# uio-bmi/compairr

Hardware: AMD Instinct MI355X
Metric: query sequences/sec for --matrix d=1, 10M-vs-10M CDR3aa (higher is better)
Workload: dtype u64; 1 GPU; synthetic 10M-vs-10M CDR3aa, d=1 substitutions only, V/J matched; queries_total=10000000, queries_this_gpu=10000000, reference_sequences=10000000, matrix_checksum=fc9769626ca2bcf2c84e8473864b8853

## Files before the change

compairr_amd/csrc/compairr_hip.hip:

```cpp
#include "context.h"
#include "kernels_sliced.h"
#include "kernels_rows.h"
#include "kernels_pairs2.h"
#include "select.h"

#include <algorithm>
#include <cmath>
#include <cstdio>
#include <cstdlib>
#include <cstring>
#include <new>
#include <mutex>
#include <string>
#include <thread>
#include <vector>

using namespace cmpr;

std::string &cmpr_create_error()
{
  static thread_local std::string e;
  return e;
}

// ... 226 lines not shown
    if (c->ring_k0[i]) (void)hipEventDestroy(c->ring_k0[i]);
    if (c->ring_km[i]) (void)hipEventDestroy(c->ring_km[i]);
    if (c->ring_k1[i]) (void)hipEventDestroy(c->ring_k1[i]);
  }
  if (c->ev_stop) (void)hipEventDestroy(c->ev_stop);
  if (c->ev_usage) (void)hipEventDestroy(c->ev_usage);
  if (c->d_usage) (void)hipFree(c->d_usage);
  if (c->h_usage) (void)hipHostFree(c->h_usage);
  c->arena_a.release();
  c->arena_b.release();
  if (c->stage_host) (void)hipHostFree(c->stage_host);
  if (c->h_sizes) (void)hipHostFree(c->h_sizes);
  for (uint32_t i = 0; i < cmpr_context::NCOPY_EV; i++)
    if (c->ev_copy[i]) (void)hipEventDestroy(c->ev_copy[i]);
  for (hipEvent_t e : c->ev_layout)
    if (e) (void)hipEventDestroy(e);
  if (c->copy_stream) (void)hipStreamDestroy(c->copy_stream);
  if (c->stream) (void)hipStreamDestroy(c->stream);
  delete c;
}

extern "C" const char *cmpr_last_error(const cmpr_context *c)
{
  return c ? c->err.c_str() : cmpr_create_error().c_str();
}

extern "C" uint32_t cmpr_rows(const cmpr_context *c) { return c ? c->R1 : 0; }
extern "C" uint32_t cmpr_cols(const cmpr_context *c) { return c ? c->R2 : 0; }

namespace {
enum TunLock { LOCK_NEVER, LOCK_REF, LOCK_QUERIES };
enum : unsigned { T_NO_PLAN = 1, T_WRITE_ONLY = 2 };

struct Tunable {
  const char *name;
  int64_t cmpr_context::*field;
  int64_t lo, hi;
  TunLock lock;
  unsigned flags;
  const char *range_msg;
  bool (*also)(const cmpr_context *, int64_t);
  void (*after)(cmpr_context *, int64_t);
  const char *lock_msg;
};

bool power_of_two(const cmpr_context *, int64_t v) { return (v & (v - 1)) == 0; }
bool not_zero(const cmpr_context *, int64_t v) { return v != 0; }
bool class_res_fits(const cmpr_context *c, int64_t v) { return v <= (int64_t)max_class_res((uint32_t)c->opt.alphabet_size); }
void force_waves(cmpr_context *c, int64_t) { c->waves_per_block_forced = true; }
void pretend_never_overflows(cmpr_context *c, int64_t v)
{
  c->force_no_redo = v != 0;
  c->usage_pending = false;
}
const char SHARD_RANGE[] = "work_shard_count must be 1..65535, work_shard_index 0..count-1",
           SHARD_LOCK[] = "set the work shard before cmpr_set_queries";
const char BOOL_RANGE[] = " must be 0 or 1", AUTO_RANGE[] = " must be -1 (auto), 0 or 1";

#define F(field) &cmpr_context::field
const Tunable TUNABLES[] = {
  {"blocks_per_cu", F(blocks_per_cu), 1, 16, LOCK_NEVER, 0, " must be 1..16"},
  {"variant", F(variant), -1, 2, LOCK_REF, 0, " must be -1 (default), 0, 1 or 2"},
  {"class_residues", F(class_residues), -1, 8, LOCK_REF, 0,
   " must be -1..4 (amino acids; four: variant 2, d = 1, else three) / -1..8 (nucleotides)", class_res_fits},
  {"class_anchor", F(class_anchor), -1, 65535, LOCK_REF, 0, " must be -1..65535"},
  {"heavy_threshold", F(heavy_threshold), -1, INT64_MAX, LOCK_REF, 0, " must be >= -1"},
  {"slice_words_log2", F(slice_words_log2), -1, 13, LOCK_REF, 0, " must be -1 (default) or 1..13", not_zero},
  {"chunk_tiles", F(chunk_tiles), 0, 512, LOCK_QUERIES, 0, " must be 0..512"},
#ifdef CMPR_ABLATION
  {"debug", F(debug), INT64_MIN, INT64_MAX, LOCK_NEVER, 0, ""},
#else
  {"debug", F(debug), 1, 0, LOCK_NEVER, 0, "the debug switches exist only in a -DCMPR_ABLATION build"},
#endif
  {"host_threads", F(host_threads), 1, 256, LOCK_NEVER, T_NO_PLAN, " must be 1..256"},
  {"table_log2_delta", F(table_log2_delta), 0, 3, LOCK_REF, 0, " must be 0..3"},
  {"part_buckets_log2", F(part_buckets_log2), 2, 30, LOCK_REF, 0, " must be 2..30"},
  {"deferred_resolve", F(deferred_resolve), 0, 1, LOCK_NEVER, 0, BOOL_RANGE},
  {"d2_pairs", F(d2_pairs), -1, 1, LOCK_REF, 0, AUTO_RANGE},
  {"d2_buffers", F(d2_buffers), 1, 2, LOCK_REF, 0, " must be 1 or 2"},
  {"chunk_deal", F(chunk_deal), 0, 1, LOCK_NEVER, 0, " must be 0 (static) or 1 (by a counter)"},
  {"narrow_upload", F(narrow_upload), -1, 1, LOCK_NEVER, T_NO_PLAN, AUTO_RANGE},
  {"item_wg", F(item_wg), 0, 1, LOCK_NEVER, T_NO_PLAN, BOOL_RANGE},
  {"layout_recompute", F(layout_recompute), 0, 1, LOCK_NEVER, T_NO_PLAN, BOOL_RANGE},
  {"layout_timing", F(layout_timing), 0, 1, LOCK_NEVER, T_NO_PLAN, BOOL_RANGE},
  {"layout_zob_lds", F(layout_zob_lds), 0, 1, LOCK_NEVER, T_NO_PLAN | T_WRITE_ONLY, BOOL_RANGE},
  {"record_tiles", F(record_tiles), 0, 2, LOCK_QUERIES, T_NO_PLAN, " must be 0, 1 or 2"},
  {"assume_never_overflows", nullptr, INT64_MIN, INT64_MAX, LOCK_NEVER, T_NO_PLAN | T_WRITE_ONLY, "", nullptr, pretend_never_overflows},
  {"dedup_tag_bits", F(dedup_tag_bits), 0, 32, LOCK_NEVER, T_NO_PLAN, " must be 0..32"},
  {"resolve_blocks_per_cu", F(resolve_blocks_per_cu), 1, 8, LOCK_NEVER, 0, " must be 1..8"},
  {"pos_segments", F(pos_segments), 1, 256, LOCK_QUERIES, 0, " must be a power of two, 1..256", power_of_two},
  {"pos_grow", F(pos_grow), -1, 1, LOCK_NEVER, 0, AUTO_RANGE},
  {"pos_capacity", F(pos_capacity), 0, INT64_MAX, LOCK_QUERIES, 0, " must be >= 0"},
  {"work_shard_count", F(work_shard_count), 1, 65535, LOCK_QUERIES, 0, SHARD_RANGE, nullptr, nullptr, SHARD_LOCK},
  {"work_shard_index", F(work_shard_index), 0, 65535, LOCK_QUERIES, 0, SHARD_RANGE, nullptr, nullptr, SHARD_LOCK},
  {"small_slice_tiles", F(small_slice_tiles), 0, 64, LOCK_QUERIES, 0, " must be 0..64"},
  {"sub2_items", F(sub2_items), -1, 1, LOCK_QUERIES, 0, " must be -1 (default), 0 or 1"},
  {"class_rows_unstaged", F(class_rows_unstaged), 0, 1, LOCK_QUERIES, 0, BOOL_RANGE},
  {"waves_per_block", F(waves_per_block), 4, 16, LOCK_QUERIES, 0, " must be 4, 8 or 16", power_of_two, force_waves},
  {"bloom_bits_log2_delta", F(bloom_log2_delta), -4, 4, LOCK_REF, 0, " must be -4..4"},
  {"slice_pages", F(slice_pages), -1, (int64_t)PAGE_E_MAX, LOCK_REF, 0, " must be -1..3"},
  {"page_budget", F(page_budget), 0, 1 << 24, LOCK_REF, 0, " must be 0..2^24"},
  {"bucket_bitmap", F(bucket_bitmap), -1, 1, LOCK_NEVER, 0, AUTO_RANGE},
  {"fill_slices", F(fill_slices), 0, 1, LOCK_REF, 0, BOOL_RANGE},
  {"direct_slices_log2", F(direct_slices_log2), -1, 12, LOCK_NEVER, 0, " must be -1 (auto) or 0..12"},
  {"row_filter_x16", F(row_filter_x16), 8, 128, LOCK_REF, 0, " must be 8..128 (sixteenths of a byte per entry)"},
};
#undef F

const Tunable *find_tunable(const char *name)
{
  for (const Tunable &t : TUNABLES)
    if (!strcmp(t.name, name))
      return &t;
  return nullptr;
}

bool in_range(const cmpr_context *c, const Tunable &t, int64_t value)
{
  return value >= t.lo && value <= t.hi && (!t.also || t.also(c, value));
}

void store_tunable(cmpr_context *c, const Tunable &t, int64_t value)
{
  if (t.field)
    c->*t.field = value;
  if (t.after)
    t.after(c, value);
}

void tunable_from_environment(cmpr_context *c, const char *variable, const char *name)
{
  const char *e = getenv(variable);
  const Tunable *t = find_tunable(name);
  if (e && t && in_range(c, *t, atoi(e)))
    store_tunable(c, *t, atoi(e));
}

}

extern "C" int cmpr_set_tunable(cmpr_context *c, const char *name, int64_t value)
{
  if (!c || !name)
    return CMPR_EINVAL;
  const Tunable *t = find_tunable(name);
  if (!t)
    return fail(c, CMPR_EINVAL, std::string("unknown tunable: ") + name);
  if (!in_range(c, *t, value))
    return fail(c, CMPR_EINVAL, t->range_msg[0] == ' ' ? t->name + std::string(t->range_msg) : t->range_msg);
  if (t->lock == LOCK_REF ? c->have_ref : t->lock == LOCK_QUERIES && c->have_q)
    return fail(c, CMPR_ESTATE, t->lock_msg ? t->lock_msg : std::string("set ") + t->name + " before " +
                                (t->lock == LOCK_REF ? "cmpr_set_reference" : "cmpr_set_queries"));
  store_tunable(c, *t, value);
  if (!(t->flags & T_NO_PLAN)) {
    invalidate_plan(c);
    c->usage_pending = c->never_overflows = false;
  }
  return CMPR_OK;
}

extern "C" int cmpr_get_tunable(cmpr_context *c, const char *name, int64_t *value)
{
  if (!c || !name || !value)
    return CMPR_EINVAL;
  std::string n(name);
  if (n == "variant") *value = c->have_ref ? (c->rows ? 2 : c->sliced ? 1 : 0) : c->variant;
  else if (n == "bloom_bits_log2_delta") {
// ... 1028 lines not shown
```

compairr_amd/csrc/context.h:

```cpp
#ifndef COMPAIRR_AMD_CONTEXT_H
#define COMPAIRR_AMD_CONTEXT_H

#include "../../include/compairr_hip.h"
#include "kernels.h"

#include "select.h"

#include <functional>
#include <map>
#include <set>
#include <string>
#include <vector>

struct SplitMix64 {
  uint64_t s;
  explicit SplitMix64(uint64_t seed) : s(seed) {}
  uint64_t next()
  {
    uint64_t z = (s += 0x9e3779b97f4a7c15ull);
    z = (z ^ (z >> 30)) * 0xbf58476d1ce4e5b9ull;
    z = (z ^ (z >> 27)) * 0x94d049bb133111ebull;
    return z ^ (z >> 31);
  }
};
// ... 54 lines not shown
  std::function<int()> finish;
};

struct RouteState {
  bool     valid = false;
  uint64_t n = 0, first_index = 0, total_records = 0;
  uint32_t n_dest = 0, record_bytes = 0;
  unsigned long long counts[64] = {};
  std::vector<double> rep_totals;
  const uint8_t  *res = nullptr;
  const uint64_t *off = nullptr, *cnt = nullptr;
  const uint32_t *v = nullptr, *j = nullptr, *rep = nullptr;
  const uint32_t *mask_lo = nullptr, *mask_hi = nullptr;
  unsigned long long *dest = nullptr;
};

struct RefPart {
  uint64_t              first = 0, n = 0;
  uint64_t              slots = 0;
  DevBuf<uint64_t>      bloom;
  DevBuf<unsigned char> rec;
  DevBuf<uint32_t>      bmap;
  void release()
  {
    bloom.release();
    rec.release();
    bmap.release();
  }
};

struct cmpr_context {
  cmpr_options opt{};
  int          device = 0;
  int          cus = 256;
  hipStream_t  stream = nullptr;
  hipEvent_t   ev_stop = nullptr;
  static const uint32_t TIME_RING = 64;
  hipEvent_t   ring_k0[TIME_RING] = {}, ring_km[TIME_RING] = {}, ring_k1[TIME_RING] = {};
  hipEvent_t   ring_start[TIME_RING] = {};
  hipEvent_t   ring_mid[TIME_RING] = {};
  uint64_t     calls = 0;
  hipEvent_t   ev_k0 = nullptr, ev_km = nullptr, ev_k1 = nullptr;
  bool         events_valid = false;
  bool         stop_is_k1 = false;
  hipEvent_t   pending_launch = nullptr;
  std::string  err;

  int64_t blocks_per_cu = 8;
  int64_t variant = -1;
  int64_t bloom_log2_delta = -100;
  int64_t row_filter_x16 = 32;
  int64_t slice_pages = -1;
  int64_t page_budget = 0;
  int64_t bucket_bitmap = -1;
  int64_t direct_slices_log2 = -1;
  int64_t fill_slices = 1;
  int64_t class_residues = -1;
  int64_t class_anchor = -1;
  int64_t heavy_threshold = -1;
  int64_t chunk_tiles = 0;
  int64_t waves_per_block = 8;
  bool    sub2_active = false;
  int64_t sub2_items = -1;
  int64_t work_shard_index = 0;
  int64_t work_shard_count = 1;
  int64_t small_slice_tiles = 0;
  int64_t class_rows_unstaged = 0;
  int64_t host_threads = 0;
  int64_t table_log2_delta = 1;
  int64_t deferred_resolve = 1;
  int64_t chunk_deal = 1;
  int64_t pos_capacity = 0;
  int64_t pos_grow = -1;
  int64_t resolve_blocks_per_cu = 5;
  int64_t pos_segments = 64;
  bool    waves_per_block_forced = false;
  int64_t debug = 0;
  int64_t slice_words_log2 = -1;
  int64_t part_buckets_log2 = 30;
  int64_t d2_pairs = -1;
  int64_t d2_buffers = 1;
  int64_t narrow_upload = -1;
  int64_t item_wg = 1, layout_recompute = 1, layout_timing = 0;
  int64_t layout_zob_lds = 1;
  int64_t record_tiles = 1;
  int64_t dedup_tag_bits = 32;
  uint32_t chunk_cap = 0;

  bool                  sliced = false;
  bool                  rows = false;
  uint32_t              npasses = 1;
  SliceGeom             geom{};
  std::vector<uint32_t> ctab;
  DevBuf<uint32_t>      d_ctab;
  DevBuf<uint32_t>      page_tab;
  uint64_t              page_slices = 0;
  DevBuf<Chunk>         chunks;
  DevBuf<cmpr::TileRef> tile_refs;
  DevBuf<uint32_t>      small_tiles;
  uint32_t              nsmall = 0;
  uint32_t              nchunks = 0;

  uint32_t          zpos = 0;
  DevBuf<uint64_t>  zob;

  bool              have_ref = false;
  uint64_t          n2 = 0;
  uint32_t          R2 = 0, longest2 = 0;
  DevBuf<uint8_t>   res2;
  DevBuf<uint64_t>  off2, cnt2, bloom;
  DevBuf<uint32_t>  v2, j2, rep2;
  DevBuf<uint32_t>  bmap2;
  DevBuf<unsigned char> rec2;
  DevBuf<uint32_t>  voff2;
  uint64_t          slots = 0, bloom_words = 0;
  uint32_t          nparts = 1;
  uint64_t          part0_n = 0;
  std::vector<RefPart> xparts;
  DevBuf<unsigned long long> stats_acc;

  bool              have_q = false;
  bool              routed = false;
  RouteState        route;
  uint64_t          n1 = 0;
  uint32_t          R1 = 0, ntiles = 0;
  DevBuf<TileDesc>  tiles;
  uint32_t          nmain_tiles = 0;
  DevBuf<uint32_t>  qres, qv, qj;
  DevBuf<uint64_t>  qgh;
  DevBuf<uint64_t>  qhins, qhdel;
  DevBuf<uint16_t>  qlen;
  DevBuf<uint32_t>  qck;
  DevBuf<cmpr::QueryRec> qrec;
  DevBuf<cmpr::ItemRec> items;
  DevBuf<uint32_t>  slice_items;
  DevBuf<cmpr::ResPack> cpk;
  DevBuf<cmpr::ResPack> qpk;
  bool              d2pairs = false;
  uint64_t          algorithmic_bytes = 0;
  double            max_cell_bound = 0;
  std::vector<double> tot1, tot2;

  DevBuf<unsigned long long> matrix;
  DevBuf<double>             matrix_f64;
  DevBuf<PosEntry>           pos_buf;
  DevBuf<unsigned long long> pos_ctr;
  unsigned long long        *ctr_cur = nullptr, *ctr_other = nullptr;
  bool                       ctr_clean = false;
  unsigned long long        *d_usage = nullptr;
  unsigned long long        *h_usage = nullptr;
  hipEvent_t                 ev_usage = nullptr;
  bool                       usage_pending = false, never_overflows = false;
  uint32_t                   usage_grid = 0, usage_nw = 0, safe_grid = 0, safe_nw = 0;
  bool                       last_without_redo = false;
  bool                       force_no_redo = false;
  bool                       async_unchecked = false, async_overflowed = false;
  hipStream_t                last_stream = nullptr;
  bool                       have_last_stream = false;
  DevArena                   arena_a, arena_b;
  void                      *stage_host = nullptr;
  size_t                     stage_host_bytes = 0;
  hipStream_t                copy_stream = nullptr;
  static const uint32_t      NCOPY_EV = 4;
  hipEvent_t                 ev_copy[NCOPY_EV] = {};
  double                     layout_upload_ms = 0, layout_tail_ms = 0, layout_total_ms = 0;
  bool                       rec_tiles = false;
// ... 159 lines not shown
```

compairr_amd/csrc/query_layout.hip:

```cpp
#include "context.h"
#include "kernels_sliced.h"

#include <hipcub/hipcub.hpp>

#include <algorithm>
#include <atomic>
#include <chrono>
#include <cstdio>
#include <cstdlib>
#include <cstring>
#include <thread>

using namespace cmpr;

namespace {

constexpr uint32_t MAXP = 1 + MAX_CLASS_RES;
constexpr uint32_t FOREIGN_SLICES_LOG2 = 12;

enum : uint32_t { VERR_OFFSETS = 1, VERR_LONG = 2, VERR_REP = 3, VERR_GENE = 4, VERR_COUNT = 5,
                  VERR_RESIDUE = 6, VERR_TOO_LONG = 7, VERR_OFFSETS0 = 8 };

struct SliceTot {
  uint32_t tiles, chunks, small, list;
// ... 804 lines not shown
    }
    for (uint32_t gl = gl_end; gl < Q.per_slice; gl++) {
      const uint32_t L = Q.longest - gl;
      const uint32_t n = c[gl];
      const uint32_t nt = (n + WAVE - 1) / WAVE;
      if (WRITE) {
        const uint64_t g = bucket * Q.per_slice + gl;
        Q.base_g[pi][g] = (tile_base + ntiles) * WAVE;
        if (pi == 0)
          Q.tfirst_g[g] = tile_base + ntiles;
      }
      for (uint32_t k = 0; k < nt; k++) {
        const uint32_t nv = min((uint32_t)WAVE, n - k * WAVE);
        if (WRITE) {
          TileDesc td;
          td.len = L;
          td.nvalid = nv;
          td.res_base = (uint32_t)(Q.res0[pi] + at.res + res);
          td.pass = pass;
          td.slice = (uint32_t)sl;
          td.k = tile_k;
          Q.tiles[tile_base + ntiles + k] = td;
        }
        res += pi == 0 ? (unsigned long long)((L + 3) / 4) * WAVE : (unsigned long long)WAVE;
        work_lens += (uint64_t)(L + 1) * nv;
      }
      ntiles += nt;
    }
  }
  uint32_t nchunks = 0, nsmall = 0, nlist = 0;
  if (Q.sliced && ntiles && sl < Q.nslices_real) {
    const uint32_t pt = (Q.rows && Q.geom.page_tab) ? Q.geom.page_tab[sl] : 0u;
    const uint32_t pe = pt & 15u;
    const uint32_t reps = 1u << pe;
    if (!Q.indels && pe == 0u && (ntiles <= Q.small_max || (pi > 0 && Q.class_unstaged))) {
      nsmall = ntiles;
      if (WRITE)
        for (uint32_t t = 0; t < ntiles; t++)
          Q.small_tiles[Q.small0[pi] + at.small + t] = tile_base + t;
    } else {
      const uint32_t nc1 = (ntiles + Q.chunk_tiles - 1) / Q.chunk_tiles;
      nchunks = nc1 * reps;
      nlist = ntiles;
      if (WRITE) {
        for (uint32_t t = 0; t < ntiles; t++) {
          TileRef r;
          r.td = Q.tiles[tile_base + t];
          r.t = tile_base + t;
          r.pad = 0;
          Q.tile_refs[Q.list0[pi] + at.list + t] = r;
        }
        for (uint32_t k = 0; k < nc1; k++)
          for (uint32_t rp = 0; rp < reps; rp++) {
            Chunk ck;
            ck.slice = page_slice(Q.geom, (uint32_t)sl, pt, rp);
            ck.first_tile = Q.list0[pi] + at.list + k * Q.chunk_tiles;
            ck.ntiles = min(Q.chunk_tiles, ntiles - k * Q.chunk_tiles);
            ck.pass = pass | (rp << CHUNK_PAGE_SHIFT) | (pe << CHUNK_PAGE_E_SHIFT);
            if (Q.sub2_items && pi == 0 && k == 0)
              ck.pass |= CHUNK_WITH_ITEMS;
            if (Q.pairs2) {
              uint32_t lmax = 0;
              for (uint32_t t = 0; t < ck.ntiles; t++)
                lmax = max(lmax, Q.tiles[tile_base + k * Q.chunk_tiles + t].len);
              ck.pass |= ((lmax + 1u) / 2u) << 16;
            }
            Q.chunks[Q.chunk0[pi] + at.chunks + k * reps + rp] = ck;
          }
      }
    }
  }
  if (!WRITE) {
    SliceTot t;
    t.tiles = ntiles;
    t.chunks = nchunks;
    t.small = nsmall;
    t.list = nlist;
    t.res = res;
    Q.tot[pi][sl] = t;
  }
  (void)work_lens;
}


template <uint32_t LAYOUT_WG, int MODE>
__global__ void __launch_bounds__(LAYOUT_WG, (LAYOUT_WG == 1024 || MODE == 0) ? 4 : 6)
scatter_kernel(const QL Q, uint64_t q0, uint64_t q1, uint32_t row0)
{
  layout_mode_assume<MODE>(Q);
  extern __shared__ uint64_t scat_lds[];
  uint64_t *const zl = scat_lds;
  uint32_t *const ctl = (uint32_t *)(zl + (Q.zob_lds ? Q.zob_pos_words : 0u));
  uint32_t *const ibase = ctl + (Q.ctab_lds ? Q.geom.off_hv : 0u);
  uint32_t *const gb = ibase + (Q.item_wg ? Q.nitem_slices : 0u);
  constexpr int NP = MODE == 0 ? OWN_NP_MAX : 3;
  const uint32_t own_np = MODE == 0 ? Q.own_np : 3u, own_dw = 4u * own_np + 1u;
  uint32_t *const wave_words = gb + (Q.group_wg ? Q.G : 0u) + (threadIdx.x & ~63u) * own_dw;
  const uint32_t lane = threadIdx.x & 63u;
  uint32_t *const mine = wave_words + lane * own_dw;
  const uint32_t *const ct = Q.ctab_lds ? ctl : Q.geom.ctab;
  const uint64_t *const zt = Q.zob_lds ? zl : Q.zob;
  if (Q.zob_lds)
    for (uint32_t k = threadIdx.x; k < Q.zob_pos_words; k += LAYOUT_WG)
      zl[k] = Q.zob[k];
  if (Q.ctab_lds)
    for (uint32_t k = threadIdx.x; k < Q.geom.off_hv; k += LAYOUT_WG)
      ctl[k] = Q.geom.ctab[k];
  if (Q.group_wg) {
    const uint32_t *const row = Q.gbase_w + (size_t)(row0 + blockIdx.x) * Q.G;
    for (uint32_t g = threadIdx.x; g < Q.G; g += LAYOUT_WG)
      gb[g] = Q.base_g[0][g] + row[g];
  }
  if (Q.zob_lds || Q.ctab_lds || Q.group_wg)
    __syncthreads();
  if (Q.item_wg) {
    const uint32_t *const row = Q.rbase + (size_t)(row0 + blockIdx.x) * Q.nitem_slices;
    for (uint32_t k = threadIdx.x; k < Q.nitem_slices; k += LAYOUT_WG)
      ibase[k] = Q.cbase[k] + row[k];
    __syncthreads();
  }
  const uint64_t total = total_of(Q);
  struct Fields {
    uint64_t b, e;
    uint32_t g, rk;
  };
  const bool want_h = Q.ngroups != 0 && Q.rows, want_ck = Q.ngroups != 0 && (Q.rows || Q.sub2_items);
  auto fetch = [&](uint64_t i) -> Fields {
    Fields f;
    f.b = f.e = 0;
    f.g = 0xffffffffu;
    f.rk = 0;
    if (i < q1) {
      f.g = Q.grp[0][i];
      f.rk = Q.rank[i];
      f.b = Q.off[i];
      f.e = Q.off[i + 1];
    }
    return f;
  };
  const uint64_t stride = (uint64_t)gridDim.x * LAYOUT_WG;
  uint64_t i0 = q0 + (uint64_t)blockIdx.x * LAYOUT_WG + (threadIdx.x & ~63u);
  Fields cur = fetch(i0 + lane);
  for (; i0 < q1; i0 += stride) {
    const uint64_t i = i0 + lane;
    uint32_t slot = 0xffffffffu;
    QueryRec qr;
    qr.cnt = 0;
    qr.v = qr.j = qr.rep = qr.len = qr.orig = 0;
    const uint32_t g = cur.g;
    const uint64_t b = cur.b, e = cur.e;
    const uint32_t rk = cur.rk;
    uint32_t gbase = 0, ck = 0;
    uint64_t h_q = 0, hins_q = 0;
    OwnPieces<NP> pieces;
    pieces.fits = false;
    if (g != 0xffffffffu) {
      gbase = LDBG(Q, LDBG_S_NO_BASE) ? 0u : Q.group_wg ? gb[g] : Q.base_g[0][g];
      pieces = own_load<NP>(Q, b, e, total, own_np);
      qr.cnt = Q.counts ? Q.cnt[i] : 1ull;
      qr.v = Q.genes ? Q.v[i] : 0u;
      qr.j = Q.genes ? Q.j[i] : 0u;
      qr.orig = Q.orig ? Q.orig[i] : (uint32_t)i;
      qr.rep = Q.existence ? qr.orig : Q.rep[i];
      if (want_h) {
        h_q = Q.h_tmp[i];
        if (Q.indels)
// ... 265 lines not shown
    return (d & m) | (padw & ~m);
  };
#pragma unroll
  for (uint32_t w = 0; w < 9; w++)
    if (w < nd)
      dst[(size_t)w * WAVE] = padded(qr.res[w], w);
  if (nd > 9) {
    const uint8_t *s = valid ? Q.res + Q.off[a.src] : Q.res;
    const uint32_t L = qr.len;
    for (uint32_t w = 9; w < nd; w++) {
      uint32_t d = 0;
#pragma unroll
      for (uint32_t k = 0; k < 4; k++)
        if (4 * w + k < L)
          d |= (uint32_t)s[4 * w + k] << (8 * k);
      dst[(size_t)w * WAVE] = padded(d, w);
    }
  }
  }
}

__global__ void __launch_bounds__(256)
item_replicas_kernel(const QL Q)
{
  const uint64_t k = (uint64_t)blockIdx.x * 256 + threadIdx.x;
  if (k >= (uint64_t)Q.nitem_slices)
    return;
  if (Q.item_wg) {
    Q.ccnt[k] = Q.ccnt_r[(size_t)k * ITEM_PAD];
    return;
  }
  uint32_t run = 0;
  for (uint32_t r = 0; r < Q.item_reps; r++) {
    const size_t rk = (size_t)r * Q.nitem_slices + k;
    Q.rbase[rk] = run;
    run += Q.ccnt_r[rk];
  }
  Q.ccnt[k] = run;
}

struct SizesBlock {
  SliceTot last_tot, last_pre;
  unsigned long long alg, sums[4];
  uint32_t verr[2];
};

__global__ void __launch_bounds__(1024)
sizes_kernel(const QL Q, const uint32_t *cpad, uint64_t ncs, unsigned long long *sums, SizesBlock *blk)
{
  typedef hipcub::BlockScan<uint32_t, 1024> Scan;
  __shared__ typename Scan::TempStorage tmp;
  unsigned long long run0 = 0, run1 = 0;
  for (uint64_t base = 0; base < ncs; base += 1024) {
    const uint64_t k = base + threadIdx.x;
    const uint32_t a = k < ncs ? cpad[k] : 0u, b = k < ncs ? Q.cnch[k] : 0u;
    uint32_t ea, eb, ta, tb;
    Scan(tmp).ExclusiveSum(a, ea, ta);
    __syncthreads();
    Scan(tmp).ExclusiveSum(b, eb, tb);
    __syncthreads();
    if (k < ncs) {
      Q.cbase[k] = (uint32_t)run0 + ea;
      Q.cchpre[k] = (uint32_t)run1 + eb;
    }
    run0 += ta;
    run1 += tb;
  }
  if (threadIdx.x == 0) {
    blk->last_tot = Q.tot[0][Q.nslices - 1];
    blk->last_pre = Q.pre[0][Q.nslices - 1];
    blk->alg = *Q.alg_bytes;
    blk->sums[0] = run0;
    blk->sums[1] = run1;
    blk->sums[2] = sums[2];
    blk->sums[3] = sums[3];
    blk->verr[0] = Q.verr[0];
    blk->verr[1] = Q.verr[1];
  }
  double *rt = (double *)(blk + 1);
  for (uint32_t r = threadIdx.x; r < Q.n_rep; r += 1024)
    rt[r] = Q.rep_total[r];
}

__global__ void __launch_bounds__(256)
item_padding_kernel(const QL Q, const uint32_t *padded, uint32_t total)
{
  const uint64_t k = (uint64_t)blockIdx.x * 256 + threadIdx.x;
  ItemRec none;
  memset(&none, 0xff, sizeof none);
  if (k < (uint64_t)Q.nitem_slices)
    for (uint32_t x = Q.cbase[k] + Q.ccnt[k]; x < Q.cbase[k] + padded[k]; x++)
      Q.items[x] = none;
  if (k < WAVE)
    Q.items[total + k] = none;
}

__device__ inline uint32_t item_slice_pages(const QL &Q, uint64_t k, uint32_t *slice, uint32_t *pt_out)
{
  if (Q.sub2_items || !Q.rows)
    return 0u;
  uint32_t gi = 0;
  for (uint32_t x = 1; x < Q.ngroups; x++)
    if (k >= Q.goff[x])
      gi = x;
  const uint32_t ls = Q.gslice0[gi] + (uint32_t)(k - Q.goff[gi]);
  const uint32_t pt = Q.geom.page_tab ? Q.geom.page_tab[ls] : 0u;
  if (slice)
    *slice = ls;
  if (pt_out)
    *pt_out = pt;
  return pt & 15u;
}

__global__ void __launch_bounds__(256)
class_pad_kernel(const QL Q, uint32_t *padded)
{
  const uint64_t k = (uint64_t)blockIdx.x * 256 + threadIdx.x;
  if (k >= (uint64_t)Q.nitem_slices)
    return;
  uint32_t blocks = (Q.ccnt[k] + WAVE - 1) / WAVE;
  padded[k] = blocks * WAVE;
  if (Q.sub2_items) {
    if (k % Q.ngroups != 0) {
      Q.cnch[k] = 0;
      return;
    }
    for (uint32_t g = 1; g < Q.ngroups; g++)
      blocks += (Q.ccnt[k + g] + WAVE - 1) / WAVE;
    if (Q.tot[0][k / Q.ngroups].chunks > 0)
      blocks = 0;
  }
  Q.cnch[k] = ((blocks + Q.cblocks - 1) / Q.cblocks) << item_slice_pages(Q, k, nullptr, nullptr);
}

__global__ void __launch_bounds__(256)
class_chunks_kernel(const QL Q)
{
  const uint64_t k = (uint64_t)blockIdx.x * 256 + threadIdx.x;
  if (k >= (uint64_t)Q.nitem_slices)
    return;
  uint32_t gi = 0;
  for (uint32_t x = 1; x < Q.ngroups; x++)
    if (k >= Q.goff[x])
      gi = x;
  uint32_t blocks = (Q.ccnt[k] + WAVE - 1) / WAVE;
  if (Q.sub2_items) {
    if (k % Q.ngroups != 0)
      return;
    for (uint32_t g = 1; g < Q.ngroups; g++)
      blocks += (Q.ccnt[k + g] + WAVE - 1) / WAVE;
    gi = 0;
    const uint32_t sl = (uint32_t)(k / Q.ngroups);
    if (Q.tot[0][sl].chunks > 0) {
      Q.slice_items[sl] = make_uint2(Q.cbase[k], blocks);
      return;
    }
    Q.slice_items[sl] = make_uint2(0u, 0u);
  }
  const uint32_t nc = (blocks + Q.cblocks - 1) / Q.cblocks;
  uint32_t ls = 0, pt = 0;
  const uint32_t pe = item_slice_pages(Q, k, &ls, &pt);
  for (uint32_t q = 0; q < nc; q++)
    for (uint32_t rp = 0; rp < (1u << pe); rp++) {
      Chunk ck;
      ck.slice = Q.sub2_items ? (uint32_t)(k / Q.ngroups) : page_slice(Q.geom, ls, pt, rp);
      ck.first_tile = Q.cbase[k] + q * Q.cblocks * WAVE;
      ck.ntiles = min(Q.cblocks, blocks - q * Q.cblocks);
      ck.pass = (3 + gi) | (rp << CHUNK_PAGE_SHIFT) | (pe << CHUNK_PAGE_E_SHIFT);
      Q.chunks[Q.cchunk0 + Q.cchpre[k] + (q << pe) + rp] = ck;
    }
}


__device__ inline bool sibling_of(const QL &Q, uint64_t g, uint32_t ip, uint32_t &sib, uint32_t &nt)
{
  const uint64_t bucket = g / Q.per_slice;
  const uint32_t gl = (uint32_t)(g % Q.per_slice);
// ... 1018 lines not shown
      HIP_TRY(c, hipEventRecord(ev, cs));
      upload_ms += std::chrono::duration<double, std::milli>(std::chrono::steady_clock::now() - t0).count();
      HIP_TRY(c, hipStreamWaitEvent(c->stream, ev, 0));
      if (narrow) {
        hipcub::TransformInputIterator<unsigned long long, Len16To64, const uint16_t *> it(
            (const uint16_t *)at(o_len16) + q0, Len16To64());
        size_t b = cub_bytes;
        HIP_TRY(c, hipcub::DeviceScan::ExclusiveScan(cub_tmp, b, it, (unsigned long long *)at(o_off) + q0,
                                                     hipcub::Sum(), (unsigned long long)r0, (int)(q1 - q0 + 1),
                                                     c->stream));
        hipLaunchKernelGGL(widen_kernel, dim3(blocks_for(q1 - q0)), dim3(256), 0, c->stream,
                           (const uint16_t *)at(o_v16), (const uint16_t *)at(o_j16), (const uint16_t *)at(o_rep16),
                           (const uint32_t *)at(o_cnt32),
                           c->opt.ignore_genes ? nullptr : (uint32_t *)at(o_v),
                           c->opt.ignore_genes ? nullptr : (uint32_t *)at(o_j), (uint32_t *)at(o_rep),
                           c->opt.ignore_counts ? nullptr : (uint64_t *)at(o_cnt), q0, q1);
        HIP_TRY(c, hipGetLastError());
      }
      hipLaunchKernelGGL(keys_fn, dim3(ranges[r].grid), dim3(LAYOUT_WG), lds, c->stream, Q, q0, q1, ranges[r].row0);
      HIP_TRY(c, hipGetLastError());
    }
    if (n == 0) {
      HIP_TRY(c, hipEventRecord(c->ev_copy[0], c->copy_stream));
      HIP_TRY(c, hipStreamWaitEvent(c->stream, c->ev_copy[0], 0));
    }
    if (!redo_wide)
      break;
    for (auto &t : workers)
      t.join();
    HIP_TRY(c, hipStreamSynchronize(c->copy_stream));
    HIP_TRY(c, hipStreamSynchronize(c->stream));
    HIP_TRY(c, hipMemsetAsync(base, 0, zero_bytes, c->stream));
    narrow = false;
    upload_ms = 0;
    if (attempt)
      return fail(c, CMPR_ESTATE, "upload did not settle");
  }
  const auto t_uploaded = std::chrono::steady_clock::now();

  if (routing) {
    uint32_t hv[2] = {0, 0};
    unsigned long long counts[64];
    std::vector<double> tot(n_rep, 0.0);
    HIP_TRY(c, hipMemcpyAsync(hv, Q.verr, sizeof hv, hipMemcpyDeviceToHost, c->stream));
    HIP_TRY(c, hipMemcpyAsync(counts, Q.dest_cnt, sizeof counts, hipMemcpyDeviceToHost, c->stream));
    if (n_rep)
      HIP_TRY(c, hipMemcpyAsync(tot.data(), Q.rep_total, n_rep * sizeof(double), hipMemcpyDeviceToHost, c->stream));
    HIP_TRY(c, hipStreamSynchronize(c->stream));
    if (hv[0] == VERR_TOO_LONG)
      return fail(c, CMPR_EINVAL, "query longer than the longest_query given to cmpr_set_reference");
    if (hv[0])
      return fail(c, hv[0] == VERR_LONG ? CMPR_EUNSUPPORTED : CMPR_EINVAL, verr_message(hv[0]));
    RouteState &R = c->route;
    R.n = n;
    R.first_index = src.first_index;
    R.n_dest = wstep;
    R.record_bytes = record_bytes;
    R.total_records = 0;
    for (uint32_t d = 0; d < 64; d++) {
      R.counts[d] = d < wstep ? counts[d] : 0;
      R.total_records += R.counts[d];
    }
    R.rep_totals = tot;
    R.res = Q.res; R.off = Q.off; R.v = Q.v; R.j = Q.j; R.rep = Q.rep; R.cnt = Q.cnt;
    R.mask_lo = Q.grp[0];
    R.mask_hi = Q.rank;
    R.dest = Q.dest_cnt;
    R.valid = true;
    c->layout_upload_ms = upload_ms;
    c->layout_total_ms = std::chrono::duration<double, std::milli>(std::chrono::steady_clock::now() - t_begin).count();
    c->layout_tail_ms = std::chrono::duration<double, std::milli>(std::chrono::steady_clock::now() - t_uploaded).count();
    if (getenv("COMPAIRR_HIP_DEBUG"))
      fprintf(stderr, "compairr_hip: route_queries %.2f ms = arena A %.2f + upload (keys hidden) %.2f + counts %.2f  "
                      "(copy calls %.2f; %llu queries, %llu records)\n", c->layout_total_ms,
              std::chrono::duration<double, std::milli>(t_arena_a - t_begin).count(),
              std::chrono::duration<double, std::milli>(t_uploaded - t_arena_a).count(), c->layout_tail_ms, upload_ms,
              (unsigned long long)n, (unsigned long long)R.total_records);
    quiesce.ok = true;
    return CMPR_OK;
  }

  const size_t slices_lds_want = (size_t)SLICES_WG * (c->sliced ? 2 : 1) * per_slice * sizeof(uint32_t);
  const size_t slices_lds = slices_lds_want <= 48 * 1024 ? slices_lds_want : 0;
  {
    SliceTot zero;
    memset(&zero, 0, sizeof zero);
    hipLaunchKernelGGL(slices_kernel<0>, dim3((uint32_t)((nslices + SLICES_WG - 1) / SLICES_WG)), dim3(SLICES_WG),
                       slices_lds, c->stream, Q, 0u, slices_lds ? 1u : 0u);
    HIP_TRY(c, hipGetLastError());
    size_t b = cub_bytes;
    HIP_TRY(c, hipcub::DeviceScan::ExclusiveScan(cub_tmp, b, Q.tot[0], Q.pre[0], SliceTotSum(), zero,
                                                 (int)nslices, c->stream));
  }
  if (ngroups) {
    hipLaunchKernelGGL(item_replicas_kernel, dim3(blocks_for(ncs)), dim3(256), 0, c->stream, Q);
    HIP_TRY(c, hipGetLastError());
    hipLaunchKernelGGL(class_pad_kernel, dim3(blocks_for(ncs)), dim3(256), 0, c->stream, Q, cpad);
    HIP_TRY(c, hipGetLastError());
  }
  if (indel_passes) {
    hipLaunchKernelGGL(sibling_count_kernel, dim3(blocks_for(G)), dim3(256), 0, c->stream, Q, G, sib_cnt);
    HIP_TRY(c, hipGetLastError());
    hipLaunchKernelGGL(sibling_chunks_kernel, dim3(blocks_for(n2s)), dim3(256), 0, c->stream,
                       sib_cnt, n2s, (uint32_t)chunk_tiles, sib_nch);
    HIP_TRY(c, hipGetLastError());
    size_t b = cub_bytes;
    HIP_TRY(c, hipcub::DeviceScan::ExclusiveSum(cub_tmp, b, sib_cnt, sib_lpre, (int)n2s, c->stream));
    b = cub_bytes;
    HIP_TRY(c, hipcub::DeviceScan::ExclusiveSum(cub_tmp, b, sib_nch, sib_cpre, (int)n2s, c->stream));
    b = cub_bytes;
    HIP_TRY(c, sum64(cub_tmp, b, sib_cnt, sums + 2, (int)n2s, c->stream));
    b = cub_bytes;
    HIP_TRY(c, sum64(cub_tmp, b, sib_nch, sums + 3, (int)n2s, c->stream));
  }
  hipLaunchKernelGGL(sizes_kernel, dim3(1), dim3(1024), 0, c->stream, Q, cpad, ngroups ? ncs : (uint64_t)0, sums,
                     (SizesBlock *)at(o_blk));
  HIP_TRY(c, hipGetLastError());
  if (c->h_sizes_bytes < blk_bytes) {
    if (c->h_sizes)
      (void)hipHostFree(c->h_sizes);
    c->h_sizes = nullptr;
    c->h_sizes_bytes = 0;
    HIP_TRY(c, hipHostMalloc(&c->h_sizes, blk_bytes + 65536, hipHostMallocDefault));
    c->h_sizes_bytes = blk_bytes + 65536;
  }
  HIP_TRY(c, hipMemcpyAsync(c->h_sizes, at(o_blk), blk_bytes, hipMemcpyDeviceToHost, c->stream));
  HIP_TRY(c, hipStreamSynchronize(c->stream));
  const SizesBlock hb = *(const SizesBlock *)c->h_sizes;
  const SliceTot last_tot = hb.last_tot, last_pre = hb.last_pre;
  const uint32_t hv[2] = {hb.verr[0], hb.verr[1]};
  const unsigned long long alg_bytes = hb.alg;
  const unsigned long long hsums[4] = {hb.sums[0], hb.sums[1], hb.sums[2], hb.sums[3]};
  {
    const double *rt = (const double *)((const SizesBlock *)c->h_sizes + 1);
    c->tot1.assign(rt, rt + n_rep);
  }
  const auto t_sizes = std::chrono::steady_clock::now();
  if (hv[0] == VERR_TOO_LONG)
    return fail(c, CMPR_EINVAL, "query longer than the longest_query given to cmpr_set_reference");
  if (hv[0])
    return fail(c, hv[0] == VERR_LONG ? CMPR_EUNSUPPORTED : CMPR_EINVAL, verr_message(hv[0]));
  c->algorithmic_bytes = alg_bytes;
  if (from_records && src.totals)
    c->tot1.assign(src.totals, src.totals + n_rep);

  {
    double m1 = 0, m2 = 0;
    for (double x : c->tot1) m1 = std::max(m1, x);
    for (double x : c->tot2) m2 = std::max(m2, x);
    c->max_cell_bound = m1 * m2;
    if (!is_f64_score(c->opt) && c->max_cell_bound >= 18446744073709551616.0 / 2)
      return fail(c, CMPR_EUNSUPPORTED,
                  "duplicate counts too large for exact 64-bit accumulation");
  }

  uint64_t ntiles = 0, nchunks = 0, nlist = 0, nsmall = 0, res_words = 0;
  {
    const SliceTotSum add;
    const SliceTot t = add(last_pre, last_tot);
    Q.tile0[0] = Q.chunk0[0] = Q.list0[0] = Q.small0[0] = 0;
    Q.res0[0] = 0;
    ntiles = t.tiles;
    nchunks = t.chunks;
    nlist = t.list;
    nsmall = t.small;
    res_words = t.res;
    c->nmain_tiles = t.tiles;
  }
  const uint64_t cslots = hsums[0], class_chunks = hsums[1];
  if (ntiles * WAVE >= 0xffffffffull)
    return fail(c, CMPR_EUNSUPPORTED, "too many query tiles");
// ... 32 lines not shown
  const size_t o_ln = cb.take((size_t)nsmall * sizeof(uint32_t));
  const size_t o_ln2 = cb.take((size_t)nsmall * sizeof(uint32_t));
  const size_t o_sout = cb.take((size_t)nsmall * sizeof(uint32_t));
  const size_t o_ssort = cb.take(small_sort_bytes + 256);
  if ((rc = arena_fit(c, c->arena_b, cb.used))) return rc;
  char *const bb = c->arena_b.base;
  Chunk *const chunks_unsorted = (Chunk *)(bb + o_chunks_u);
  Q.aux = (QAux *)(bb + o_aux);

  c->ntiles = (uint32_t)ntiles;
  c->nchunks = (uint32_t)nchunks;
  c->nsmall = (uint32_t)nsmall;
  if ((rc = dev_reserve(c, c->tiles, (size_t)ntiles))) return rc;
  if ((rc = dev_reserve(c, c->chunks, (size_t)nchunks))) return rc;
  if ((rc = dev_reserve(c, c->tile_refs, (size_t)nlist))) return rc;
  if ((rc = dev_reserve(c, c->small_tiles, (size_t)nsmall))) return rc;
  if ((rc = dev_reserve(c, c->qres, (size_t)res_words + 9 * WAVE))) return rc;
  if ((rc = dev_reserve(c, c->qlen, slots))) return rc;
  if ((rc = dev_reserve(c, c->qrec, slots))) return rc;
  HIP_TRY(c, hipMemsetAsync(c->qres.p + res_words, 0, 9 * WAVE * sizeof(uint32_t), c->stream));
  if (!c->opt.ignore_genes && !c->rows) {
    if ((rc = dev_reserve(c, c->qv, slots))) return rc;
    if ((rc = dev_reserve(c, c->qj, slots))) return rc;
  } else {
    c->qv.release();
    c->qj.release();
  }
  if (!c->opt.ignore_genes || c->rows || (!c->sliced && c->opt.differences == 0)) {
    if ((rc = dev_reserve(c, c->qgh, slots))) return rc;
  } else {
    c->qgh.release();
  }
  if (c->rows) {
    if ((rc = dev_reserve(c, c->qck, slots))) return rc;
  } else {
    c->qck.release();
  }
  if (c->d2pairs) {
    if ((rc = dev_reserve(c, c->qpk, slots))) return rc;
  } else {
    c->qpk.release();
  }
  if (c->rows && c->opt.indels) {
    if ((rc = dev_reserve(c, c->qhins, slots))) return rc;
    if ((rc = dev_reserve(c, c->qhdel, slots))) return rc;
  } else {
    c->qhins.release();
    c->qhdel.release();
  }
  bool pad_items = false;
  if (ngroups) {
    const size_t ni = (size_t)cslots + WAVE;
    if ((rc = dev_reserve(c, c->items, ni))) return rc;
    pad_items = true;
    if (sub2_items) {
      if ((rc = dev_reserve(c, c->cpk, ni))) return rc;
      if ((rc = dev_reserve(c, c->slice_items, 2 * (size_t)nslices_real))) return rc;
      HIP_TRY(c, hipMemsetAsync(c->slice_items.p, 0, 2 * (size_t)nslices_real * sizeof(uint32_t), c->stream));
    } else if (c->d2pairs) {
      if ((rc = dev_reserve(c, c->cpk, ni))) return rc;
      c->slice_items.release();
    } else {
      c->cpk.release();
      c->slice_items.release();
    }
  } else {
    c->items.release();
    c->cpk.release();
    c->slice_items.release();
  }
  const auto t_reserved = std::chrono::steady_clock::now();
  Q.tiles = c->tiles.p;
  Q.chunks = chunks_unsorted;
  Q.tile_refs = c->tile_refs.p;
  Q.small_tiles = c->small_tiles.p;
  Q.cpk = c->cpk.p;
  Q.qpk = c->qpk.p;
  Q.slice_items = (uint2 *)c->slice_items.p;
  Q.qres = c->qres.p; Q.qv = c->qv.p; Q.qj = c->qj.p;
  Q.qck = c->qck.p; Q.qgh = c->qgh.p; Q.qhins = c->qhins.p;
  Q.qhdel = c->qhdel.p; Q.qlen = c->qlen.p; Q.qrec = c->qrec.p;
  Q.items = c->items.p;

  if (pad_items) {
    hipLaunchKernelGGL(item_padding_kernel, dim3(blocks_for(std::max<uint64_t>(ncs, WAVE))), dim3(256), 0, c->stream, Q,
                       cpad, (uint32_t)cslots);
    HIP_TRY(c, hipGetLastError());
  }
  hipLaunchKernelGGL(slices_kernel<1>, dim3((uint32_t)((nslices + SLICES_WG - 1) / SLICES_WG)), dim3(SLICES_WG),
                     slices_lds, c->stream, Q, 0u, slices_lds ? 1u : 0u);
  HIP_TRY(c, hipGetLastError());
  LAYOUT_MARK(2);
  if (n) {
    for (const Range &g : ranges) {
      hipLaunchKernelGGL(scatter_fn, dim3(g.grid), dim3(LAYOUT_WG), scatter_lds, c->stream, Q, g.q0, g.q1, g.row0);
      HIP_TRY(c, hipGetLastError());
    }
  }
  LAYOUT_MARK(3);
  c->rec_tiles = rows_rec;
  c->rec_hash = c->rec_tiles && rec_hash;
  if (ntiles && !c->rec_tiles) {
    const size_t fill_lds = Q.recompute ? (zob_lds ? zob_words * sizeof(uint64_t) : 0) + ctab_bytes : 0;
    const int fo = occupancy_of(c, (const void *)fill_tiles_kernel, 256, fill_lds);
    const uint32_t fgrid = (uint32_t)std::min<uint64_t>((ntiles + 3) / 4, (uint64_t)c->cus * (uint64_t)std::max(fo, 1));
    hipLaunchKernelGGL(fill_tiles_kernel, dim3(fgrid), dim3(256), fill_lds, c->stream, Q, (uint32_t)ntiles);
    HIP_TRY(c, hipGetLastError());
  }
  LAYOUT_MARK(4);
  if (ngroups) {
    hipLaunchKernelGGL(class_chunks_kernel, dim3(blocks_for(ncs)), dim3(256), 0, c->stream, Q);
    HIP_TRY(c, hipGetLastError());
  }
  if (indel_passes) {
    hipLaunchKernelGGL(sibling_fill_kernel, dim3(blocks_for(G)), dim3(256), 0, c->stream, Q, G,
                       sib_lpre, sib_fill, (uint32_t)main_list);
    HIP_TRY(c, hipGetLastError());
    hipLaunchKernelGGL(sibling_write_chunks_kernel, dim3(blocks_for(2 * nslices)), dim3(256), 0,
                       c->stream, Q, sib_cnt, sib_lpre, sib_cpre, (uint32_t)main_list,
                       (uint32_t)main_chunks);
    HIP_TRY(c, hipGetLastError());
  }

  const bool select_share = wstep > 1 && !place_mine;
  if (nchunks && nchunks <= ORDER_MAX && !select_share) {
    uint32_t *wk = (uint32_t *)(bb + o_wk);
    HIP_TRY(c, hipMemsetAsync(wk + nchunks, 0, sizeof(uint32_t), c->stream));
    hipLaunchKernelGGL(chunk_work_kernel, dim3(blocks_for(nchunks)), dim3(256), 0, c->stream, Q,
                       (uint32_t)nchunks, wk, (uint32_t *)nullptr);
    hipLaunchKernelGGL(chunk_order_kernel, dim3(1), dim3(1024), 0, c->stream, Q, (uint32_t)nchunks, wk, c->chunks.p);
    HIP_TRY(c, hipGetLastError());
    c->nchunks = (uint32_t)nchunks;
  } else if (nchunks) {
    uint32_t *wk = (uint32_t *)(bb + o_wk), *wk2 = (uint32_t *)(bb + o_wk2);
    uint32_t *ix = (uint32_t *)(bb + o_ix), *ix2 = (uint32_t *)(bb + o_ix2);
    hipLaunchKernelGGL(chunk_work_kernel, dim3(blocks_for(nchunks)), dim3(256), 0, c->stream, Q,
                       (uint32_t)nchunks, wk, ix);
    HIP_TRY(c, hipGetLastError());
    size_t sb = sort_bytes;
    HIP_TRY(c, hipcub::DeviceRadixSort::SortPairsDescending(bb + o_sort, sb, wk, wk2, ix, ix2, (int)nchunks, 0, 32,
                                                            c->stream));
    uint64_t mine = nchunks;
    const uint32_t *order = ix2;
    Tmp<uint32_t> sel;
    if (select_share) {
      if ((rc = select_mine(c, ix2, (uint32_t)nchunks, sel, mine, [&](unsigned char *flag) {
            hipLaunchKernelGGL(chunk_mine_kernel, dim3(blocks_for(nchunks)), dim3(256), 0, c->stream,
                               chunks_unsorted, ix2, (uint32_t)nchunks, wfirst, wstep, flag);
          })))
        return rc;
      order = sel.b.p;
    }
    if (mine)
      hipLaunchKernelGGL(gather_chunks_kernel, dim3(blocks_for(mine)), dim3(256), 0, c->stream,
                         chunks_unsorted, order, (uint32_t)mine, c->chunks.p);
    HIP_TRY(c, hipGetLastError());
    if (select_share)
      HIP_TRY(c, hipStreamSynchronize(c->stream));
    c->nchunks = (uint32_t)mine;
  }
  if (nsmall) {
    uint32_t *ln = (uint32_t *)(bb + o_ln), *ln2 = (uint32_t *)(bb + o_ln2), *out = (uint32_t *)(bb + o_sout);
    hipLaunchKernelGGL(small_len_kernel, dim3(blocks_for(nsmall)), dim3(256), 0, c->stream, Q,
                       (uint32_t)nsmall, ln);
    HIP_TRY(c, hipGetLastError());
    size_t sb = small_sort_bytes;
    HIP_TRY(c, hipcub::DeviceRadixSort::SortPairsDescending(bb + o_ssort, sb, ln, ln2, c->small_tiles.p, out,
                                                            (int)nsmall, 0, 17, c->stream));
    uint64_t mine = nsmall;
    const uint32_t *keep = out;
    Tmp<uint32_t> sel;
    if (select_share) {
      if ((rc = select_mine(c, out, (uint32_t)nsmall, sel, mine, [&](unsigned char *flag) {
            hipLaunchKernelGGL(small_mine_kernel, dim3(blocks_for(nsmall)), dim3(256), 0, c->stream, Q,
// ... 81 lines not shown
```

Measured before the change: 6.010 billion query sequences/s.

## Add wave-per-slice walk kernel for slice layout and fold item padding into it

Adds a slice_walk_kernel that gives each slice to one wavefront, using wave prefix sums to compute tile, residue and chunk offsets cooperatively across lanes instead of the per-thread slices_kernel. The write pass also absorbs the item padding work into extra blocks of the same launch, removing one kernel launch. It is enabled by default through a new layout_chain option, with the old path kept behind the switch. This targets query-layout preprocessing time, which may be a small share of the end-to-end throughput, and it duplicates layout logic that must stay consistent with the original kernel.

```diff
diff --git a/compairr_amd/csrc/compairr_hip.hip b/compairr_amd/csrc/compairr_hip.hip
--- a/compairr_amd/csrc/compairr_hip.hip
+++ b/compairr_amd/csrc/compairr_hip.hip
@@ -332,6 +332,7 @@
   {"narrow_upload", F(narrow_upload), -1, 1, LOCK_NEVER, T_NO_PLAN, AUTO_RANGE},
   {"item_wg", F(item_wg), 0, 1, LOCK_NEVER, T_NO_PLAN, BOOL_RANGE},
   {"layout_recompute", F(layout_recompute), 0, 1, LOCK_NEVER, T_NO_PLAN, BOOL_RANGE},
+  {"layout_chain", F(layout_chain), 0, 1, LOCK_NEVER, T_NO_PLAN, BOOL_RANGE},
   {"layout_timing", F(layout_timing), 0, 1, LOCK_NEVER, T_NO_PLAN, BOOL_RANGE},
   {"layout_zob_lds", F(layout_zob_lds), 0, 1, LOCK_NEVER, T_NO_PLAN | T_WRITE_ONLY, BOOL_RANGE},
   {"record_tiles", F(record_tiles), 0, 2, LOCK_QUERIES, T_NO_PLAN, " must be 0, 1 or 2"},
diff --git a/compairr_amd/csrc/context.h b/compairr_amd/csrc/context.h
--- a/compairr_amd/csrc/context.h
+++ b/compairr_amd/csrc/context.h
@@ -160,6 +160,7 @@
   int64_t d2_buffers = 1;
   int64_t narrow_upload = -1;
   int64_t item_wg = 1, layout_recompute = 1, layout_timing = 0;
+  int64_t layout_chain = 1;
   int64_t layout_zob_lds = 1;
   int64_t record_tiles = 1;
   int64_t dedup_tag_bits = 32;
diff --git a/compairr_amd/csrc/query_layout.hip b/compairr_amd/csrc/query_layout.hip
--- a/compairr_amd/csrc/query_layout.hip
+++ b/compairr_amd/csrc/query_layout.hip
@@ -910,6 +910,234 @@
   (void)work_lens;
 }
 
+constexpr uint32_t WALK_WG = 256;
+constexpr uint32_t WALK_OWN = 4;
+
+__device__ inline void item_padding_of(const QL &Q, const uint32_t *padded, uint32_t total, uint64_t k);
+
+__device__ inline uint32_t wave_incl_sum(uint32_t x, uint32_t lane)
+{
+#pragma unroll
+  for (uint32_t o = 1; o < (uint32_t)WAVE; o <<= 1) {
+    const uint32_t y = (uint32_t)__shfl_up((int)x, o, WAVE);
+    if (lane >= o)
+      x += y;
+  }
+  return x;
+}
+
+__device__ inline unsigned long long wave_incl_sum64(unsigned long long x, uint32_t lane)
+{
+#pragma unroll
+  for (uint32_t o = 1; o < (uint32_t)WAVE; o <<= 1) {
+    const unsigned long long y = (unsigned long long)__shfl_up((long long)x, o, WAVE);
+    if (lane >= o)
+      x += y;
+  }
+  return x;
+}
+
+struct WalkRun {
+  uint32_t tstart, tcnt;
+  uint32_t L, c;
+  uint32_t shared;
+  unsigned long long rstart;
+};
+
+__device__ inline WalkRun walk_run_of_lane(const WalkRun &r, uint32_t src)
+{
+  WalkRun q;
+  q.tstart = (uint32_t)__shfl((int)r.tstart, (int)src, WAVE);
+  q.tcnt = (uint32_t)__shfl((int)r.tcnt, (int)src, WAVE);
+  q.L = (uint32_t)__shfl((int)r.L, (int)src, WAVE);
+  q.c = (uint32_t)__shfl((int)r.c, (int)src, WAVE);
+  q.shared = (uint32_t)__shfl((int)r.shared, (int)src, WAVE);
+  q.rstart = (unsigned long long)__shfl((long long)r.rstart, (int)src, WAVE);
+  return q;
+}
+
+template <typename F>
+__device__ inline void walk_runs(uint32_t lane, const WalkRun &r, uint32_t n, F f)
+{
+  for (uint32_t i = 0; i < n && i < WALK_OWN; i++)
+    f(r, i);
+  unsigned long long big = __ballot(n > WALK_OWN);
+  while (big) {
+    const uint32_t src = (uint32_t)__builtin_ctzll(big);
+    big &= big - 1ull;
+    const WalkRun q = walk_run_of_lane(r, src);
+    const uint32_t nq = (uint32_t)__shfl((int)n, (int)src, WAVE);
+    for (uint32_t i = WALK_OWN + lane; i < nq; i += (uint32_t)WAVE)
+      f(q, i);
+  }
+}
+
+template <int WRITE>
+__global__ void __launch_bounds__(WALK_WG)
+slice_walk_kernel(const QL Q, uint32_t pi, uint32_t slice_blocks, const uint32_t *cpad, uint32_t items_total)
+{
+  if (blockIdx.x >= slice_blocks) {
+    if (WRITE)
+      item_padding_of(Q, cpad, items_total, (uint64_t)(blockIdx.x - slice_blocks) * WALK_WG + threadIdx.x);
+    return;
+  }
+  const uint32_t lane = threadIdx.x & (uint32_t)(WAVE - 1);
+  const uint64_t sl = (uint64_t)blockIdx.x * (WALK_WG / WAVE) + threadIdx.x / WAVE;
+  if (sl >= Q.nslices)
+    return;
+  const uint32_t nhv = Q.sliced ? 2u : 1u;
+  const uint32_t pass = pi == 0 ? 0u : 2u + pi;
+  const uint32_t *const cnt = Q.cnt_g[pi] + sl * nhv * Q.per_slice;
+  const uint32_t gl_end = Q.longest >= Q.min_mixed ? min(Q.per_slice, Q.longest - Q.min_mixed + 1u) : 0u;
+  SliceTot at;
+  at.tiles = at.chunks = at.small = at.list = 0;
+  at.res = 0;
+  if (WRITE)
+    at = Q.pre[pi][sl];
+  const uint32_t tile_base = Q.tile0[pi] + at.tiles;
+
+  const bool one = Q.per_slice <= (uint32_t)WAVE;
+  uint32_t cp0 = 0, cp1 = 0;
+  if (one && lane < Q.per_slice) {
+    cp0 = cnt[lane];
+    if (nhv > 1u)
+      cp1 = cnt[Q.per_slice + lane];
+  }
+  const uint32_t pt_of_slice = (Q.sliced && Q.rows && Q.geom.page_tab && sl < Q.nslices_real) ? Q.geom.page_tab[sl] : 0u;
+
+  uint32_t ntiles = 0, h1 = 0, lh1 = 0;
+  unsigned long long res = 0;
+  uint32_t nl0 = 0, nl1 = 0;
+  uint32_t mode = 0, reps = 1, pe = 0, pt = 0;
+
+  auto sweep = [&](const bool emit) {
+    uint32_t tiles_run = 0;
+    unsigned long long res_run = 0;
+    for (uint32_t hv = 0; hv < nhv; hv++) {
+      const uint32_t hv_start = tiles_run, nl = hv ? nl1 : nl0;
+      uint32_t nlong_run = 0;
+      bool seen = false;
+      for (uint32_t g0 = 0; g0 < Q.per_slice; g0 += (uint32_t)WAVE) {
+        const uint32_t gl = g0 + lane;
+        const bool valid = gl < Q.per_slice;
+        const uint32_t c = !valid ? 0u : one ? (hv ? cp1 : cp0) : cnt[hv * Q.per_slice + gl];
+        const bool sh = valid && gl < gl_end;
+        const uint32_t cs = sh ? c : 0u;
+        const uint32_t incl = nlong_run + wave_incl_sum(cs, lane), excl = incl - cs;
+        WalkRun r;
+        r.tcnt = sh ? (incl + 63u) / 64u - (excl + 63u) / 64u : (c + 63u) / 64u;
+        r.L = valid ? Q.longest - gl : 0u;
+        r.c = c;
+        r.shared = sh ? 1u : 0u;
+        const unsigned long long rw = pi == 0 ? (unsigned long long)((r.L + 3u) / 4u) * WAVE : (unsigned long long)WAVE;
+        const uint32_t tincl = wave_incl_sum(r.tcnt, lane);
+        r.tstart = tiles_run + tincl - r.tcnt;
+        const unsigned long long rmine = (unsigned long long)r.tcnt * rw, rincl = wave_incl_sum64(rmine, lane);
+        r.rstart = res_run + rincl - rmine;
+        if (hv == 1u && !seen) {
+          const unsigned long long some = __ballot(r.tcnt > 0u);
+          if (some) {
+            lh1 = Q.longest - (g0 + (uint32_t)__builtin_ctzll(some));
+            seen = true;
+          }
+        }
+        if (WRITE && emit) {
+          if (valid) {
+            const uint64_t g = (sl * nhv + hv) * Q.per_slice + gl;
+            Q.base_g[pi][g] = sh ? (uint32_t)((uint64_t)(tile_base + hv_start) * WAVE + excl) : (tile_base + r.tstart) * WAVE;
+            if (pi == 0)
+              Q.tfirst_g[g] = sh ? tile_base + hv_start + excl / WAVE : tile_base + r.tstart;
+          }
+          walk_runs(lane, r, r.tcnt, [&](const WalkRun &q, uint32_t i) {
+            const uint32_t t = q.tstart + i;
+            const unsigned long long qrw = pi == 0 ? (unsigned long long)((q.L + 3u) / 4u) * WAVE : (unsigned long long)WAVE;
+            TileDesc td;
+            td.len = q.L;
+            td.nvalid = q.shared ? min((uint32_t)WAVE, nl - (t - hv_start) * WAVE) : min((uint32_t)WAVE, q.c - i * WAVE);
+            td.res_base = (uint32_t)(Q.res0[pi] + at.res + q.rstart + i * qrw);
+            td.pass = pass;
+            td.slice = (uint32_t)sl;
+            td.k = hv ? Q.geom.k : 0u;
+            Q.tiles[tile_base + t] = td;
+            if (mode == 1u)
+              Q.small_tiles[Q.small0[pi] + at.small + t] = tile_base + t;
+            if (mode == 2u) {
+              TileRef ref;
+              ref.td = td;
+              ref.t = tile_base + t;
+              ref.pad = 0;
+              Q.tile_refs[Q.list0[pi] + at.list + t] = ref;
+            }
+          });
+          if (mode == 2u) {
+            const uint32_t ct = Q.chunk_tiles;
+            const uint32_t kfirst = (r.tstart + ct - 1u) / ct, kend = (r.tstart + r.tcnt + ct - 1u) / ct;
+            walk_runs(lane, r, r.tcnt ? kend - kfirst : 0u, [&](const WalkRun &q, uint32_t i) {
+              const uint32_t k = (q.tstart + ct - 1u) / ct + i;
+              const uint32_t first = k * ct, n_here = min(ct, ntiles - first);
+              uint32_t word = pass | (pe << CHUNK_PAGE_E_SHIFT);
+              if (Q.sub2_items && pi == 0 && k == 0u)
+                word |= CHUNK_WITH_ITEMS;
+              if (Q.pairs2) {
+                const uint32_t lmax = (first < h1 && h1 < first + n_here) ? max(q.L, lh1) : q.L;
+                word |= ((lmax + 1u) / 2u) << 16;
+              }
+              for (uint32_t rp = 0; rp < reps; rp++) {
+                Chunk ck;
+                ck.slice = page_slice(Q.geom, (uint32_t)sl, pt, rp);
+                ck.first_tile = Q.list0[pi] + at.list + first;
+                ck.ntiles = n_here;
+                ck.pass = word | (rp << CHUNK_PAGE_SHIFT);
+                Q.chunks[Q.chunk0[pi] + at.chunks + k * reps + rp] = ck;
+              }
+            });
+          }
+        }
+        tiles_run += (uint32_t)__shfl((int)tincl, WAVE - 1, WAVE);
+        res_run += (unsigned long long)__shfl((long long)rincl, WAVE - 1, WAVE);
+        nlong_run = (uint32_t)__shfl((int)incl, WAVE - 1, WAVE);
+      }
+      if (!emit) {
+        if (hv)
+          nl1 = nlong_run;
+        else
+          nl0 = nlong_run;
+        if (hv == 0u)
+          h1 = tiles_run;
+      }
+    }
+    ntiles = tiles_run;
+    res = res_run;
+  };
+
+  sweep(false);
+  uint32_t nchunks = 0, nsmall = 0, nlist = 0;
+  if (Q.sliced && ntiles && sl < Q.nslices_real) {
+    pt = pt_of_slice;
+    pe = pt & 15u;
+    reps = 1u << pe;
+    if (!Q.indels && pe == 0u && (ntiles <= Q.small_max || (pi > 0 && Q.class_unstaged))) {
+      mode = 1u;
+      nsmall = ntiles;
+    } else {
+      mode = 2u;
+      nchunks = (ntiles + Q.chunk_tiles - 1u) / Q.chunk_tiles * reps;
+      nlist = ntiles;
+    }
+  }
+  if (WRITE) {
+    sweep(true);
+  } else if (lane == 0u) {
+    SliceTot t;
+    t.tiles = ntiles;
+    t.chunks = nchunks;
+    t.small = nsmall;
+    t.list = nlist;
+    t.res = res;
+    Q.tot[pi][sl] = t;
+  }
+}
+
 
 template <uint32_t LAYOUT_WG, int MODE>
 __global__ void __launch_bounds__(LAYOUT_WG, (LAYOUT_WG == 1024 || MODE == 0) ? 4 : 6)
@@ -1341,10 +1569,8 @@
     rt[r] = Q.rep_total[r];
 }
 
-__global__ void __launch_bounds__(256)
-item_padding_kernel(const QL Q, const uint32_t *padded, uint32_t total)
-{
-  const uint64_t k = (uint64_t)blockIdx.x * 256 + threadIdx.x;
+__device__ inline void item_padding_of(const QL &Q, const uint32_t *padded, uint32_t total, uint64_t k)
+{
   ItemRec none;
   memset(&none, 0xff, sizeof none);
   if (k < (uint64_t)Q.nitem_slices)
@@ -1352,6 +1578,12 @@
       Q.items[x] = none;
   if (k < WAVE)
     Q.items[total + k] = none;
+}
+
+__global__ void __launch_bounds__(256)
+item_padding_kernel(const QL Q, const uint32_t *padded, uint32_t total)
+{
+  item_padding_of(Q, padded, total, (uint64_t)blockIdx.x * 256 + threadIdx.x);
 }
 
 __device__ inline uint32_t item_slice_pages(const QL &Q, uint64_t k, uint32_t *slice, uint32_t *pt_out)
@@ -2536,11 +2768,17 @@
 
   const size_t slices_lds_want = (size_t)SLICES_WG * (c->sliced ? 2 : 1) * per_slice * sizeof(uint32_t);
   const size_t slices_lds = slices_lds_want <= 48 * 1024 ? slices_lds_want : 0;
+  const bool chain = c->layout_chain != 0;
+  const uint32_t walk_blocks = (uint32_t)((nslices + WALK_WG / WAVE - 1) / (WALK_WG / WAVE));
   {
     SliceTot zero;
     memset(&zero, 0, sizeof zero);
-    hipLaunchKernelGGL(slices_kernel<0>, dim3((uint32_t)((nslices + SLICES_WG - 1) / SLICES_WG)), dim3(SLICES_WG),
-                       slices_lds, c->stream, Q, 0u, slices_lds ? 1u : 0u);
+    if (chain)
+      hipLaunchKernelGGL(slice_walk_kernel<0>, dim3(walk_blocks), dim3(WALK_WG), 0, c->stream, Q, 0u, walk_blocks,
+                         (const uint32_t *)nullptr, 0u);
+    else
+      hipLaunchKernelGGL(slices_kernel<0>, dim3((uint32_t)((nslices + SLICES_WG - 1) / SLICES_WG)), dim3(SLICES_WG),
+                         slices_lds, c->stream, Q, 0u, slices_lds ? 1u : 0u);
     HIP_TRY(c, hipGetLastError());
     size_t b = cub_bytes;
     HIP_TRY(c, hipcub::DeviceScan::ExclusiveScan(cub_tmp, b, Q.tot[0], Q.pre[0], SliceTotSum(), zero,
@@ -2739,14 +2977,21 @@
   Q.qhdel = c->qhdel.p; Q.qlen = c->qlen.p; Q.qrec = c->qrec.p;
   Q.items = c->items.p;
 
-  if (pad_items) {
-    hipLaunchKernelGGL(item_padding_kernel, dim3(blocks_for(std::max<uint64_t>(ncs, WAVE))), dim3(256), 0, c->stream, Q,
-                       cpad, (uint32_t)cslots);
+  if (chain) {
+    const uint32_t pad_blocks = pad_items ? (uint32_t)((std::max<uint64_t>(ncs, WAVE) + WALK_WG - 1) / WALK_WG) : 0u;
+    hipLaunchKernelGGL(slice_walk_kernel<1>, dim3(walk_blocks + pad_blocks), dim3(WALK_WG), 0, c->stream, Q, 0u,
+                       walk_blocks, (const uint32_t *)cpad, (uint32_t)cslots);
     HIP_TRY(c, hipGetLastError());
-  }
-  hipLaunchKernelGGL(slices_kernel<1>, dim3((uint32_t)((nslices + SLICES_WG - 1) / SLICES_WG)), dim3(SLICES_WG),
-                     slices_lds, c->stream, Q, 0u, slices_lds ? 1u : 0u);
-  HIP_TRY(c, hipGetLastError());
+  } else {
+    if (pad_items) {
+      hipLaunchKernelGGL(item_padding_kernel, dim3(blocks_for(std::max<uint64_t>(ncs, WAVE))), dim3(256), 0, c->stream, Q,
+                         cpad, (uint32_t)cslots);
+      HIP_TRY(c, hipGetLastError());
+    }
+    hipLaunchKernelGGL(slices_kernel<1>, dim3((uint32_t)((nslices + SLICES_WG - 1) / SLICES_WG)), dim3(SLICES_WG),
+                       slices_lds, c->stream, Q, 0u, slices_lds ? 1u : 0u);
+    HIP_TRY(c, hipGetLastError());
+  }
   LAYOUT_MARK(2);
   if (n) {
     for (const Range &g : ranges) {
```

Measured after the change: 6.178 billion query sequences/s, median of 6. 1.03x the previous value.
